# matsengrp/linearham

Hardware: AMD Instinct MI355X
Metric: phylo-HMM log-likelihood evals/sec (100-leaf x 400-site family) (higher is better)
Workload: dtype f64

## Files before the change

linearham_amd/csrc/lh_asr.hip:

```cpp
#include <cstdlib>

#include "lh_device.h"

namespace lh {

namespace {

__device__ __forceinline__ void philox_round(uint32_t& c0, uint32_t& c1, uint32_t& c2, uint32_t& c3, uint32_t k0,
                                             uint32_t k1) {
  const uint64_t p0 = (uint64_t)0xD2511F53u * c0, p1 = (uint64_t)0xCD9E8D57u * c2;
  const uint32_t hi0 = (uint32_t)(p0 >> 32), lo0 = (uint32_t)p0;
  const uint32_t hi1 = (uint32_t)(p1 >> 32), lo1 = (uint32_t)p1;
  const uint32_t n0 = hi1 ^ c1 ^ k0, n2 = hi0 ^ c3 ^ k1;
  c0 = n0;
  c1 = lo1;
  c2 = n2;
  c3 = lo0;
}

__device__ __forceinline__ double asr_uniform(uint64_t seed, uint64_t sample, uint32_t site, uint32_t draw) {
  uint32_t c0 = site, c1 = draw, c2 = (uint32_t)sample, c3 = (uint32_t)(sample >> 32);
  uint32_t k0 = (uint32_t)seed, k1 = (uint32_t)(seed >> 32);
#pragma unroll
  for (int r = 0; r < 10; ++r) {
// ... 190 lines not shown
  uint8_t* flags = st_stack + 16 * 256;
  int32_t* misc = reinterpret_cast<int32_t*>(flags + (((size_t)R * NP + 15) & ~(size_t)15));

  const int tid = threadIdx.x;
  const int lane = tid & 63;
  const int wave = __builtin_amdgcn_readfirstlane(tid >> 6);
  const int n_waves = blockDim.x >> 6;
  const int rate = blockIdx.x;
  const int sample = blockIdx.y;
  const uint64_t sample_id = sample0 + (uint64_t)sample;
  const AsrOp* __restrict__ dsc = desc + (size_t)sample * n_ops;
  const uint8_t* __restrict__ ch = choice_g + (size_t)sample * L;

  for (int i = tid; i < R * NP; i += blockDim.x) flags[i] = 0;
  __syncthreads();
  for (int j = tid; j < L; j += blockDim.x) flags[(int)ch[j] * NP + min(site_pat[j], n_prune)] = 1;
  __syncthreads();

  if (wave == n_waves - 1) {
    int run = 0;
    for (int j0 = 0; j0 < L; j0 += 64) {
      const int j = j0 + lane;
      const int c = j < L ? (int)ch[j] : 255;
      const unsigned long long mine = __ballot(c == rate);
      if (c == rate) list[run + __popcll(mine & ((1ull << lane) - 1ull))] = j;
      run += __popcll(mine);
    }
    int base = 0, prun = 0;
    for (int k = 0; k <= rate; ++k) {
      int cntk = 0;
      for (int p0 = 0; p0 < NP; p0 += 64) {
        const int p = p0 + lane;
        const bool f = p < NP && flags[k * NP + p] != 0;
        const unsigned long long m = __ballot(f);
        if (k == rate && f) {
          const int pos = cntk + __popcll(m & ((1ull << lane) - 1ull));
          plist[pos] = p;
          pslot[p] = pos;
        }
        cntk += __popcll(m);
      }
      if (k < rate)
        base += (cntk + 7) & ~7;
      else
        prun = cntk;
    }
    if (lane == 0) {
      misc[0] = run;
      misc[1] = base;
      misc[2] = prun;
    }
  }

  const double* __restrict__ e = eig + (size_t)sample * 36;
  const double rt = rates[(size_t)sample * R + rate];
  const double* __restrict__ bl = brlen + (size_t)sample * (2 * (size_t)T - 2);
  {
    double P[4][4];
    for (int j = tid; j < T + n_ops - 1; j += blockDim.x) {
      if (j < T) {
        compute_pmatrix(e, bl[j] * rt, P);
        double* o = tiptab + j * 16;
#pragma unroll
        for (int i = 0; i < 4; ++i)
#pragma unroll
          for (int st = 0; st < 4; ++st) o[st * 4 + i] = P[i][st];
      } else {
        const int k = j - T;
        compute_pmatrix(e, bl[T + dsc[k].b.z] * rt, P);
        double* o = pin + (size_t)k * 16;
#pragma unroll
        for (int i = 0; i < 4; ++i)
#pragma unroll
          for (int q = 0; q < 4; ++q) o[i * 4 + q] = P[i][q];
      }
    }
  }
  __syncthreads();
  const int cnt = misc[0], base = misc[1], cntp = misc[2];
  if (cnt == 0) return;

  const double* __restrict__ p4 = pi + (size_t)sample * 4;
  const uint8_t* __restrict__ nv = naive + (size_t)sample * L;
  const size_t plane = (size_t)Lp;
  double2* clv_s = clv + (size_t)sample * n_ops * 2 * plane;
  uint8_t* anc_s = anc + (size_t)sample * n_ops * (size_t)L;
  uint8_t* my_stack = st_stack + tid;

  {
    const int per = 64;
    for (int s0 = wave * per; s0 < cntp; s0 += n_waves * per) {
      const int slot = min(s0 + min(lane, per - 1), cntp - 1);
      const int pat = plist[slot];
      const int gslot = base + slot;
      const bool all_n = pat >= n_prune;
      const unsigned upat = all_n ? 0u : (unsigned)pat;
      const double2* cbase = clv_s + gslot;
      double a[4] = {1.0, 1.0, 1.0, 1.0};
      struct Up {
        int4 da, db;
        int sa, sb;
      };
      Up ring[4];
      double2 ylo[2], yhi[2];
      auto tips = [&](Up& p) {
        p.sa = msa[(unsigned)(p.da.y * n_prune) + upat];
        p.sb = msa[(unsigned)(p.da.z * n_prune) + upat];
// ... 151 lines not shown
```

linearham_amd/csrc/lh_capi.hip:

```cpp
#include <algorithm>
#include <map>
#include <cstdio>
#include <cstring>
#include <atomic>
#include <chrono>
#include <string>
#include <thread>
#include <vector>

#include "lh_device.h"

namespace lh {
const DebugOptions& debug_options() {
  static const DebugOptions opts = [] {
    DebugOptions o;
    auto set = [](const char* name) { return std::getenv(name) != nullptr; };
    auto num = [](const char* name, int dflt) { const char* e = std::getenv(name); return e ? std::atoi(e) : dflt; };
    o.chunk = std::max(256, num("LH_CHUNK", o.chunk));
    o.host_sub = std::max(256, num("LH_HOST_SUB", o.host_sub));
    o.k2b_no_pair = set("LH_K2B_NO_PAIR");
    o.k2b_vd_single = set("LH_K2B_VD_SINGLE");
    o.sample_timing = set("LH_SAMPLE_TIMING");
    o.k1_tile_cap = num("LH_K1_TILE_CAP", 0);
    o.k1_cxx_walk = set("LH_K1_CXX_WALK");
// ... 317 lines not shown
  auto cols = [&](const int32_t* src, size_t rows, size_t n, size_t n_pad, size_t inner) {
    std::vector<int32_t> t = pad_genes<int32_t>(src, rows, n, n_pad, inner, -1);
    for (int32_t& x : t) x = x >= 0 ? remap[x] : n_jcols;
    return t;
  };
  std::vector<double> ltr = pad_genes<double>(j.left_trans, W, nL, pL, 1, 0.0);
  for (size_t l = 0; l < nL; ++l) ltr[l] = j.enter_trans[l];
  std::vector<double> ntt(pR * 16, 0.0);
  for (size_t r = 0; r < nR; ++r)
    for (int a = 0; a < 4; ++a)
      for (int b = 0; b < 4; ++b) ntt[r * 16 + b * 4 + a] = j.right_ntt[r * 16 + a * 4 + b];
  if (upload_vec(f, pad_genes<double>(j.enter_lo, 1, nL, pL, 1, 0.0), &d->enter_lo)) return 1;
  if (upload_vec(f, ltr, &d->left_trans)) return 1;
  if (upload_vec(f, pad_genes<double>(j.left_lo, W, nL, pL, 1, 0.0), &d->left_lo)) return 1;
  if (upload_vec(f, cols(j.left_xmsa, W, nL, pL, 1), &d->left_xmsa)) return 1;
  if (upload_vec(f, pad_genes<double>(j.right_gp_nli, 1, nR, pR, 4, 0.0), &d->right_gp_nli)) return 1;
  if (upload_vec(f, ntt, &d->right_ntt)) return 1;
  if (upload_vec(f, pad_genes<double>(j.right_nlo, W, nR, pR, 4, 0.0), &d->right_nlo)) return 1;
  if (upload_vec(f, pad_genes<double>(j.right_trans, W, nR, pR, 1, 0.0), &d->right_trans)) return 1;
  if (upload_vec(f, pad_genes<double>(j.right_gp_li, W, nR, pR, 1, 0.0), &d->right_gp_li)) return 1;
  if (upload_vec(f, cols(j.right_xmsa, W, nR, pR, 1), &d->right_xmsa)) return 1;
  if (upload_vec(f, cols(j.nti_xmsa, W, nR, pR, 4), &d->nti_xmsa)) return 1;
  if (upload_vec(f, pad_genes<double>(j.exit_nlo, 1, nR, pR, 4, 0.0), &d->exit_nlo)) return 1;
  if (upload_vec(f, pad_genes<double>(j.exit_trans, 1, nR, pR, 1, 0.0), &d->exit_trans)) return 1;
  if (upload_vec(f, pad_genes<double>(j.exit_gp_li, 1, nR, pR, 1, 0.0), &d->exit_gp_li)) return 1;
  std::vector<int32_t> row_pat(W, f->host.n_prune);
  if (xmsa_site)
    for (size_t i = 0; i < W; ++i) row_pat[i] = pat_of_site[xmsa_site[j.nti_xmsa[i * nR * 4]]];
  if (upload_vec(f, row_pat, &d->row_pat)) return 1;
  return 0;
}

size_t k1_bytes_per_sample(const lh_family* f, int T, int R) {
  const lh::PruneWsSizes z = lh::prune_ws_sizes(T, f->host.msa_mixed_n != 0);
  const size_t n_ops = (size_t)std::max(T - 2, 1);
  return sizeof(double) * R * z.scratch_doubles_per_rate + n_ops * (sizeof(int2) + sizeof(double)) +
         z.tabs_per_sample * sizeof(int4) + sizeof(int4);
}

int ensure_workspace(lh_family* f, int n, int R, int T) {
  Workspace& w = f->ws;
  if (n <= w.n_cap && R == w.R && T == w.T) return 0;
  void** bufs[] = {(void**)&w.rates,         (void**)&w.eig,        (void**)&w.site_lik,   (void**)&w.site_scal,
                   (void**)&w.prune.scratch, (void**)&w.prune.wops, (void**)&w.prune.wlen, (void**)&w.prune.tabs,
                   (void**)&w.prune.hdr};
  for (void** b : bufs) {
    if (*b) LH_HIP(hipFree(*b));
    *b = nullptr;
  }
  w.n_cap = 0;
  const size_t L = f->host.n_prune;
  const int cap = std::max(n, 1);
  LH_HIP(hipMalloc((void**)&w.rates, sizeof(double) * cap * R));
  LH_HIP(hipMalloc((void**)&w.eig, sizeof(double) * cap * 36));
  const lh::PruneWsSizes z = lh::prune_ws_sizes(T, f->host.msa_mixed_n != 0);
  const size_t n_ops = (size_t)std::max(T - 2, 1);
  LH_HIP(hipMalloc((void**)&w.prune.scratch, sizeof(double) * cap * R * z.scratch_doubles_per_rate));
  LH_HIP(hipMalloc((void**)&w.prune.wops, sizeof(int2) * cap * n_ops));
  LH_HIP(hipMalloc((void**)&w.prune.wlen, sizeof(double) * cap * n_ops));
  LH_HIP(hipMalloc((void**)&w.prune.tabs, sizeof(int4) * cap * z.tabs_per_sample));
  LH_HIP(hipMalloc((void**)&w.prune.hdr, sizeof(int4) * cap));
  w.prune.err_flag = f->err_flag;
  LH_HIP(hipMalloc((void**)&w.site_lik, sizeof(double) * cap * R * 5 * std::max(L, (size_t)1)));
  LH_HIP(hipMalloc((void**)&w.site_scal, sizeof(int32_t) * cap * R * std::max(L, (size_t)1)));
  w.n_cap = cap;
  w.R = R;
  w.T = T;
  return 0;
}

int stage(lh_family* f, int slot, size_t bytes, void** out) {
  Staging& s = f->st;
  if (bytes > s.cap[slot]) {
    if (s.ptr[slot]) LH_HIP(hipFree(s.ptr[slot]));
    s.ptr[slot] = nullptr;
    s.cap[slot] = 0;
    LH_HIP(hipMalloc(&s.ptr[slot], bytes));
    s.cap[slot] = bytes;
  }
  *out = s.ptr[slot];
  return 0;
}

static const int kChunk = lh::debug_options().chunk;

int run_forward(lh_family* f, int n, int R, const double* site_lik, const int32_t* site_scal, const double* pi,
                const double* em_in, double* em_out, double* loglik_dev, const lh_eval_outputs* outs,
                size_t sample_offset, hipStream_t stream) {
  double* fwd = (outs && outs->forward) ? outs->forward + sample_offset * f->host.forward_size : nullptr;
  int32_t* sco =
      (outs && outs->scaler_counts) ? outs->scaler_counts + sample_offset * f->host.scaler_size : nullptr;
  ForwardWs& w = f->fws;
  if (n > w.n_cap) {
    LH_HIP(hipDeviceSynchronize());
    void** bufs[] = {(void**)&w.gem, (void**)&w.jem, (void**)&w.gcnt, (void**)&w.jrs, (void**)&w.dxf, (void**)&w.dxc};
    for (void** b : bufs) {
      if (*b) LH_HIP(hipFree(*b));
      *b = nullptr;
    }
    w.n_cap = 0;
    LH_HIP(hipMalloc((void**)&w.jrs, sizeof(int32_t) * (size_t)n * std::max(f->host.vd.n_rows + f->host.dj.n_rows, 1)));
    LH_HIP(hipMalloc((void**)&w.dxf, sizeof(double) * (size_t)n * 32));
    LH_HIP(hipMalloc((void**)&w.dxc, sizeof(int32_t) * (size_t)n));
    LH_HIP(hipMalloc((void**)&w.gem, sizeof(double) * (size_t)n * std::max<int64_t>(f->host.gem_size, 1)));
    LH_HIP(hipMalloc((void**)&w.jem, sizeof(double) * (size_t)n * std::max(f->host.n_jcols, 1)));
    LH_HIP(hipMalloc((void**)&w.gcnt, sizeof(int32_t) * (size_t)n * 3));
    w.n_cap = n;
// ... 1208 lines not shown
```

linearham_amd/csrc/lh_device.h:

```cpp
#pragma once
#include <hip/hip_runtime.h>
#include <stdint.h>

#include "linearham_amd.h"

namespace lh {

constexpr double kScaleFactor = 0x1p256;
constexpr double kScaleThreshold = 0x1p-256;
constexpr double kLogScaleFactor = 177.445678223345993274;

enum : int { OP_CHERRY = 0, OP_TIP_ACC = 1, OP_POP_ACC = 2, OP_PUSH_FLAG = 16, OP_RANK_SHIFT = 8 };

enum : int { W_CHERRY = 0, W_TIP_ACC = 1, W_POP = 2, W_CTIP = 3, W_CTAB_ACC = 4 };

struct PruneWs {
  double* scratch;
  int2* wops;
  double* wlen;
  int4* tabs;
  int4* hdr;
  int32_t* err_flag;
};
struct PruneWsSizes {
// ... 50 lines not shown
  DevJunction vd, dj;
  int32_t max_genes;
  int32_t n_jcols;
  const int32_t* jcols;
  int64_t gem_size;
  int64_t forward_size;
  int64_t scaler_size;
};

__device__ static inline double fast_rcp(double v) {
  double r = __builtin_amdgcn_rcp(v);
  r = fma(fma(-v, r, 1.0), r, r);
  r = fma(fma(-v, r, 1.0), r, r);
  return r;
}

struct DevSampleJunction {
  int32_t n_rows, n_left, n_right, n_states;
  int32_t right_first_block;
  const int32_t* state_class;
  const int32_t* left_rows;
  const int32_t* left_dense;
  const double* left_lo;
  const double* left_trans;
  const double* enter_lo;
  const int32_t* right_dense;
  const int32_t* right_first;
  const double* gp;
  const double* nli;
  const double* ntt;
  const double* nlo;
  const double* li;
  const double* rtrans;
  const double* exit_nlo;
  const double* exit_trans;
  const double* exit_li;
  const double* prod;
};

struct DevSampler {
  int32_t has_d, n_v, n_d, n_j, states_per_sample, words_per_sample;
  DevSampleJunction vd, dj;
};

void launch_sample(const DevSampler& smp, const DevSampler* smp_dev, int n, const double* fwd, size_t forward_size, const uint32_t* words,
                   int words_per_sample, int32_t* states, hipStream_t stream);

void launch_posterior(const DevSampler* smp_dev, int n, double* post, size_t forward_size, const double* loglik,
                      hipStream_t stream);
int posterior_slabs(int n);
void launch_posterior_reduce(int n, size_t forward_size, const double* post, const double* loglik, const double* log_offset,
                             double* w, double* partial, double* weighted_sum, double* stats, hipStream_t stream);

__device__ static inline void compute_pmatrix(const double* __restrict__ e, double tr, double P[4][4]) {
  double ex[4];
#pragma unroll
  for (int k = 1; k < 4; ++k) ex[k] = expm1(e[k] * tr);
#pragma unroll
  for (int i = 0; i < 4; ++i)
#pragma unroll
    for (int j = 0; j < 4; ++j) {
      double v = (i == j) ? 1.0 : 0.0;
#pragma unroll
      for (int k = 1; k < 4; ++k) v = fma(e[4 + i * 4 + k] * ex[k], e[20 + k * 4 + j], v);
      P[i][j] = fmax(v, 0.0);
    }
}


void launch_model_setup(int n, int R, const double* er, const double* pi, const double* alpha,
                        double* rates, double* eig, hipStream_t stream);

int launch_prune(const DevFamily& fam, int n, int R, int T, int max_depth, const int32_t* ops,
                 const double* brlen, const double* rates, const double* eig, const PruneWs& ws, const double* pi,
                 double* site_lik, int32_t* site_scal, hipStream_t stream, bool allow_fused = true);
const char* prune_last_form();
const char* prune_last_error();

void launch_gtr_setup(int n, const double* er, const double* pi, double* eig, hipStream_t stream);

int launch_asr(const DevFamily& fam, int n, int R, int T, const int32_t* ops, const double* brlen, const double* rates,
               const double* eig, const double* pi, const double* site_lik, const int32_t* site_scal,
               const uint8_t* naive, uint64_t seed, uint64_t sample0, double* clv, void* desc, uint8_t* anc,
               uint8_t* rate_choice, const int4* hdr , hipStream_t stream);
size_t asr_desc_bytes(int T);
size_t asr_lds_bytes(int T, int L, int R, int n_prune);
size_t asr_slots(int L, int R);

void launch_forward(const DevFamily& fam, const DevFamily* fam_dev, int n, int R, const double* site_lik,
                    const int32_t* site_scal, const double* pi, const double* em_in, double* em_out, double* gem,
                    int32_t* gcnt, double* jem,
                    int32_t* jrs, double* dxf, int32_t* dxc, double* loglik, double* forward_out, int32_t* scaler_out,
                    bool extended, hipStream_t stream);
size_t forward_lds_bytes(const DevFamily& fam);

struct DebugOptions {
  int chunk = 49152;
  int host_sub = 12288;
  bool k2b_no_pair = false;
  bool k2b_vd_single = false;
  bool sample_timing = false;
  int k1_tile_cap = 0;
  bool k1_cxx_walk = false;
  bool k1_tables = false;
  bool k1_stack = false;
  bool k1_no_tables = false;
  bool k1_segments = false;
  int k1_seg_waves = 4;
  bool k1_no_fuse = false;
};
const DebugOptions& debug_options();

}
```

linearham_amd/csrc/lh_model.hip:

```cpp
#include "lh_device.h"

namespace lh {



__device__ static double gamma_p(double a, double x, double lga) {
  if (!(x > 0.0)) return 0.0;
  const double pre = exp(-x + a * log(x) - lga);
  if (x < a + 1.0) {
    double ap = a, del = fast_rcp(a), sum = del;
    for (int n = 0; n < 2000; ++n) {
      ap += 1.0;
      del *= x * fast_rcp(ap);
      sum += del;
      if (fabs(del) < fabs(sum) * 1e-17) break;
    }
    return sum * pre;
  }
  const double FPMIN = 1e-300;
  double b = x + 1.0 - a, c = 1.0 / FPMIN, d = fast_rcp(b), h = d;
  for (int i = 1; i < 2000; ++i) {
    const double an = -i * (i - a);
    b += 2.0;
    d = an * d + b;
// ... 95 lines not shown
  for (int sweep = 0; sweep < 40; ++sweep) {
    double off = 0.0;
    for (int i = 0; i < 4; ++i)
      for (int j = i + 1; j < 4; ++j) off += A[i][j] * A[i][j];
    if (off < 1e-300) break;
#pragma unroll
    for (int pp = 0; pp < 3; ++pp) {
#pragma unroll
      for (int q = pp + 1; q < 4; ++q) {
        const double apq = A[pp][q];
        if (fabs(apq) < 1e-300) continue;
        const double theta = (A[q][q] - A[pp][pp]) / (2.0 * apq);
        const double t = ((theta >= 0.0) ? 1.0 : -1.0) / (fabs(theta) + sqrt(theta * theta + 1.0));
        const double c = 1.0 / sqrt(t * t + 1.0), sn = t * c;
#pragma unroll
        for (int k = 0; k < 4; ++k) {
          const double akp = A[k][pp], akq = A[k][q];
          A[k][pp] = c * akp - sn * akq;
          A[k][q] = sn * akp + c * akq;
        }
#pragma unroll
        for (int k = 0; k < 4; ++k) {
          const double apk = A[pp][k], aqk = A[q][k];
          A[pp][k] = c * apk - sn * aqk;
          A[q][k] = sn * apk + c * aqk;
        }
#pragma unroll
        for (int k = 0; k < 4; ++k) {
          const double wkp = W[k][pp], wkq = W[k][q];
          W[k][pp] = c * wkp - sn * wkq;
          W[k][q] = sn * wkp + c * wkq;
        }
      }
    }
  }
  double lam[4] = {A[0][0], A[1][1], A[2][2], A[3][3]};
#pragma unroll
  for (int k = 3; k >= 1; --k) {
    bool up = true;
#pragma unroll
    for (int j = 0; j < k; ++j) up = up && lam[k] > lam[j];
    if (up) {
      const double t = lam[k];
      lam[k] = lam[k - 1];
      lam[k - 1] = t;
#pragma unroll
      for (int i = 0; i < 4; ++i) {
        const double w = W[i][k];
        W[i][k] = W[i][k - 1];
        W[i][k - 1] = w;
      }
    }
  }
  double* o = eig + (size_t)s * 36;
  o[0] = 0.0;
  for (int k = 1; k < 4; ++k) o[k] = lam[k];
  for (int i = 0; i < 4; ++i)
    for (int k = 0; k < 4; ++k) {
      o[4 + i * 4 + k] = W[i][k] / sq[i];
      o[20 + k * 4 + i] = W[i][k] * sq[i];
    }
}

__global__ void __launch_bounds__(256) finalize_rates_kernel(int n, int R, double* __restrict__ rates) {
  const int s = blockIdx.x * blockDim.x + threadIdx.x;
  if (s >= n) return;
  double* r = rates + (size_t)s * R;
  double prev = 0.0;
  for (int k = 0; k < R - 1; ++k) {
    const double cum = r[k];
    r[k] = (cum - prev) * R;
    prev = cum;
  }
  r[R - 1] = (1.0 - prev) * R;
}

void launch_model_setup(int n, int R, const double* er, const double* pi, const double* alpha,
                        double* rates, double* eig, hipStream_t stream) {
  const long long total = (long long)n * R;
  hipLaunchKernelGGL(model_setup_kernel, dim3((unsigned)((total + 63) / 64)), dim3(64), 0, stream, n, R, er, pi,
                     alpha, rates, eig);
  hipLaunchKernelGGL(finalize_rates_kernel, dim3((n + 255) / 256), dim3(256), 0, stream, n, R, rates);
}

void launch_gtr_setup(int n, const double* er, const double* pi, double* eig, hipStream_t stream) {
  hipLaunchKernelGGL(model_setup_kernel, dim3((unsigned)((n + 63) / 64)), dim3(64), 0, stream, n, 1, er, pi,
                     (const double*)nullptr, (double*)nullptr, eig);
}

}
```

linearham_amd/csrc/lh_prune.hip:

```cpp
#include <cstdlib>

#include <cstdio>

#include "lh_device.h"

namespace lh {

namespace {

thread_local char g_prune_form[64] = "";
thread_local char g_prune_error[256] = "";

#define LH_SLOT_COPY(dst, src)                       \
  _Pragma("unroll") for (int s_ = 0; s_ < S; ++s_) { \
    dst[s_][0] = src[s_][0];                         \
    dst[s_][1] = src[s_][1];                         \
    dst[s_][2] = src[s_][2];                         \
    dst[s_][3] = src[s_][3];                         \
  }
#define LH_PUSH_IF(d)                                   \
  if constexpr (kDepth > d) {                           \
    if (push_mask & (1u << d)) { LH_SLOT_COPY(st##d, a) } \
  }
#define LH_POP_CASE(d)          \
// ... 491 lines not shown
          a[s][0] *= kScaleFactor;
          a[s][1] *= kScaleFactor;
          a[s][2] *= kScaleFactor;
          a[s][3] *= kScaleFactor;
          ++scal[s];
        }
      }
    }
  }
  close_naive_branch<S>(a, scal, naive_tab, p4, lik, scl);
}

#undef LH_SLOT_COPY
#undef LH_PUSH_IF
#undef LH_POP_CASE
#undef LH_POP_SLOT
#undef LH_DECL

}

template <int kDepth, bool kTwo, bool kN, bool kFused, bool kSeg = false>
__device__ __forceinline__ void prune_body(int sample, int n2, int tile, int R, int wpr, const uint8_t* __restrict__ msa, int L,
                                           int T, int n_ops, const int32_t* __restrict__ ops,
                                           const int4* __restrict__ hdr, int32_t* err_flag,
                                           const double* __restrict__ brlen, const double* __restrict__ rates,
                                           const double* __restrict__ eig, double* pmat_w, size_t rate_stride,
                                           const double* __restrict__ pi,
                                           double* __restrict__ site_lik, int32_t* __restrict__ site_scal) {
  extern __shared__ double2 smem2[];
  const int tid = threadIdx.x;
  const int wave_all = __builtin_amdgcn_readfirstlane(tid >> 6);
  const int rate = kFused ? wave_all / wpr : (int)blockIdx.y;
  const int wave = kFused ? wave_all - rate * wpr : wave_all;
  const int nthr = kFused ? wpr * 64 : (int)blockDim.x;
  const int rtid = kFused ? tid - rate * nthr : tid;
  if (hdr != nullptr && hdr[sample].w != 0) {
    const int planes = kFused ? 1 : R, plane = kFused ? 0 : rate;
    const int t0 = blockIdx.x * tile, t1 = min(t0 + tile, L);
    for (int site = t0 + tid; site < t1; site += blockDim.x) {
      for (int b = 0; b < 5; ++b) site_lik[(((size_t)sample * planes + plane) * 5 + b) * (size_t)L + site] = __builtin_nan("");
      site_scal[((size_t)sample * planes + plane) * (size_t)L + site] = 0;
    }
    return;
  }
  const size_t pm_off = ((size_t)sample * R + rate) * rate_stride;
  double* tiptab = reinterpret_cast<double*>(smem2) + (kFused ? (size_t)rate * T * 16 : 0);
  const double* naive_tab = kSeg ? tiptab + 2 * kSegOps * 16 : tiptab;
  double* ones = reinterpret_cast<double*>(smem2) + (kSeg ? (size_t)(2 * kSegOps + 1) * 16 : (size_t)(kFused ? R : 1) * T * 16);
  const int ones_off = (int)(ones - tiptab);
  if (kN && tid < 4) ones[tid] = 1.0;
  const int4* __restrict__ op_ptr = reinterpret_cast<const int4*>(ops) + (size_t)sample * n_ops;

  {
    const double* __restrict__ e = eig + (size_t)sample * 36;
    const double rt = rates[(size_t)sample * R + rate];
    const double* __restrict__ bl = brlen + (size_t)sample * (2 * (size_t)T - 2);
    double* pw = pmat_w + pm_off;
    double P[4][4];
    if constexpr (kFused) {
      uint16_t* mat_list = reinterpret_cast<uint16_t*>(reinterpret_cast<double*>(smem2) + (size_t)R * T * 16 + (kN ? 4 : 0));
      const int nodes = 2 * T - 2;
      if (rate == 0) {
        for (int k = rtid; k < n_ops; k += nthr) {
          const int4 op = op_ptr[k];
          const int kind = op.x & 15, rank = op.x >> OP_RANK_SHIFT;
          if (kind == OP_CHERRY) continue;
          mat_list[rank] = (uint16_t)(2 * k);
          if (kind == OP_POP_ACC) mat_list[rank + 1] = (uint16_t)(2 * k + 1);
        }
      }
      __syncthreads();
      const int n_inner = T - 3;
      for (int it = rtid; it < n_inner + T; it += nthr) {
        if (it < n_inner) {
          const int code = mat_list[it], k = min(code >> 1, n_ops - 1);
          const int4 op = op_ptr[k];
          const int node = min(max((code & 1) ? op.y : op.z, 0), nodes - 1);
          compute_pmatrix(e, bl[node] * rt, P);
          double* o = pw + (size_t)k * 32 + (code & 1) * 16;
#pragma unroll
          for (int i = 0; i < 4; ++i)
#pragma unroll
            for (int q = 0; q < 4; ++q) o[i * 4 + q] = P[i][q];
        } else {
          const int j = it - n_inner;
          compute_pmatrix(e, bl[j] * rt, P);
          double* o = tiptab + j * 16;
#pragma unroll
          for (int i = 0; i < 4; ++i)
#pragma unroll
            for (int st = 0; st < 4; ++st) o[st * 4 + i] = P[i][st];
        }
      }
    } else {
    const int half = nthr >= 128 ? (nthr / 128) * 64 : 0;
    const bool do_ops = half == 0 || rtid < half;
    const bool do_tips = half == 0 || rtid >= half;
    if (do_ops) {
      const int stride = half ? half : nthr;
      for (int k = rtid; k < n_ops; k += stride) {
        const int4 op = op_ptr[k];
        const int kind = op.x & 15;
        if (kind == OP_CHERRY) continue;
        double* o = pw + (size_t)k * 32;
        compute_pmatrix(e, bl[op.z] * rt, P);
#pragma unroll
        for (int i = 0; i < 4; ++i)
#pragma unroll
          for (int q = 0; q < 4; ++q) o[i * 4 + q] = P[i][q];
        if (kind == OP_POP_ACC) {
          compute_pmatrix(e, bl[op.y] * rt, P);
#pragma unroll
          for (int i = 0; i < 4; ++i)
#pragma unroll
            for (int q = 0; q < 4; ++q) o[16 + i * 4 + q] = P[i][q];
        }
      }
    }
    if (do_tips) {
      const int stride = half ? nthr - half : nthr;
      for (int j = half ? rtid - half : rtid; j < (kSeg ? 1 : T); j += stride) {
        compute_pmatrix(e, bl[j] * rt, P);
        double* o = kSeg ? tiptab + 2 * kSegOps * 16 : tiptab + j * 16;
#pragma unroll
        for (int i = 0; i < 4; ++i)
#pragma unroll
          for (int st = 0; st < 4; ++st) o[st * 4 + i] = P[i][st];
      }
    }
    }
  }
  SegCtx seg{eig + (size_t)sample * 36, brlen + (size_t)sample * (2 * (size_t)T - 2),
             rates[(size_t)sample * R + rate], tiptab, rtid, nthr};
  if constexpr (kSeg) seg_fill(seg, op_ptr, n_ops, 0);
  asm volatile("s_waitcnt vmcnt(0)" ::: "memory");
  __threadfence_block();
  __syncthreads();

  const pmat_ptr pm = pmat_after_barrier(pmat_w + pm_off);
  const int lane = tid & 63;
  const int tile0 = blockIdx.x * tile;
  const int site_end = min(tile0 + tile, L);
  const double* __restrict__ p4 = pi + (size_t)sample * 4;
  double lik[2][5];
  int scl[2] = {0, 0};
  int site0, n_own;
  bool two_sites = false;
  if constexpr (kTwo) two_sites = wave < n2;
  if (two_sites) {
    site0 = tile0 + wave * 128 + lane;
    n_own = 2;
    if constexpr (kTwo)
      prune_wave<kDepth, 2, kN, kSeg>(site0, site_end, msa, L, n_ops, op_ptr, pm, tiptab, naive_tab, ones_off, p4, lik, scl, seg);
  } else {
    site0 = tile0 + n2 * 128 + (wave - n2) * 64 + lane;
    n_own = 1;
    double lik1[1][5];
    int scl1[1];
    prune_wave<kDepth, 1, kN, kSeg>(site0, site_end, msa, L, n_ops, op_ptr, pm, tiptab, naive_tab, ones_off, p4, lik1, scl1, seg);
#pragma unroll
    for (int b = 0; b < 5; ++b) lik[0][b] = lik1[0][b];
    scl[0] = scl1[0];
  }

  if constexpr (!kFused) {
    double* lik_out = site_lik + (((size_t)sample * R + rate) * 5) * (size_t)L;
    int32_t* scal_out = site_scal + ((size_t)sample * R + rate) * (size_t)L;
#pragma unroll
    for (int s = 0; s < 2; ++s) {
      const int site = site0 + 64 * s;
      if (s < n_own && site < site_end) {
#pragma unroll
        for (int b = 0; b < 5; ++b) lik_out[(size_t)b * L + site] = lik[s][b];
        scal_out[site] = scl[s];
      }
    }
  } else {
    const int pad = n2 * 128 + (wpr - n2) * 64;
    __syncthreads();
    double* X = reinterpret_cast<double*>(smem2);
    int* SC = reinterpret_cast<int*>(X + (size_t)R * 5 * pad);
#pragma unroll
    for (int s = 0; s < 2; ++s) {
      const int idx = site0 + 64 * s - tile0;
      if (s < n_own && idx < pad) {
// ... 191 lines not shown
      const int up = __shfl_up(incl, d), dup = __shfl_up(dincl, d);
      if (lane >= d) incl += up, dincl += dup;
    }
    const int depth = depth0 + dincl - dl;
    if (in && push && op.w != depth) ok = false;
    if (in && kind == OP_POP_ACC && op.w != depth - 1) ok = false;
    if (check_ranks && in && kind != OP_CHERRY && rank != carry + incl - m) ok = false;
    if (in && !ok) bad = true;
    carry += __shfl(incl, 63);
    depth0 += __shfl(dincl, 63);
  }
  if (carry != T - 3 || depth0 != 0) bad = true;
  const bool any_bad = __builtin_amdgcn_ballot_w64(bad) != 0;
  if (lane == 0) {
    hdr[smp] = make_int4(0, 0, 0, any_bad ? 1 : 0);
    if (any_bad) atomicOr(err_flag, 1);
  }
}

template <int kDepth, bool kN, bool kFused, bool kAsm = false>
__device__ __forceinline__ void prune_body_ct(int n2, int tile, int R, int wpr, const uint8_t* __restrict__ msa,
                                              const uint64_t* __restrict__ planes, int L,
                                              int T, const int2* __restrict__ wops, const double* __restrict__ wlen,
                                              const int4* __restrict__ tabs, int tabs_stride,
                                              const int4* __restrict__ hdr, const double* __restrict__ brlen,
                                              const double* __restrict__ rates, const double* __restrict__ eig,
                                              double* pmat_w, size_t rate_stride, const double* __restrict__ pi,
                                              double* __restrict__ site_lik, int32_t* __restrict__ site_scal) {
  extern __shared__ double2 smem2[];
  constexpr int SY = kN ? 5 : 4, E = SY * SY;
  const int tid = threadIdx.x;
  const int wave_all = __builtin_amdgcn_readfirstlane(tid >> 6);
  const int rate = kFused ? wave_all / wpr : (int)blockIdx.y;
  const int wave = kFused ? wave_all - rate * wpr : wave_all;
  const int nthr = kFused ? wpr * 64 : (int)blockDim.x;
  const int rtid = kFused ? tid - rate * nthr : tid;
  const int sample = blockIdx.z;
  const int n_ops = T - 2;
  const int4 h = hdr[sample];
  const int n_w = __builtin_amdgcn_readfirstlane(h.x);
  const int n_mat = __builtin_amdgcn_readfirstlane(h.y), n_tab = __builtin_amdgcn_readfirstlane(h.z);
  const bool malformed = h.w != 0;
  double* pw = pmat_w + ((size_t)sample * R + rate) * rate_stride;
  double* ctab = pw + (size_t)(T - 3 > 0 ? T - 3 : 0) * 16;
  constexpr int kS = 2;
  double* tiptab = reinterpret_cast<double*>(smem2) + (kFused ? (size_t)rate * T * 16 : 0);
  const double* naive_tab = tiptab;
  double* ones = reinterpret_cast<double*>(smem2) + (size_t)(kFused ? R : 1) * T * 16;
  const int ones_off = (int)(ones - tiptab);
  if (kN && tid < 4) ones[tid] = 1.0;
  const int4* __restrict__ tl = tabs + (size_t)sample * tabs_stride;
  WalkOp* desc = reinterpret_cast<WalkOp*>(reinterpret_cast<double*>(smem2) + (size_t)(kFused ? R : 1) * T * 16 + (kN ? 4 : 0));
  for (int i = tid; i < n_w; i += blockDim.x) desc[i] = wops[(size_t)sample * n_ops + i];

  const int n_q = min(n_tab, nthr >> 2);
  const bool pc_lane = (rtid & 3) == 0 && (rtid >> 2) < n_q;
  int4 tcell = make_int4(1, 1, 0, 0);
  if ((rtid >> 2) < n_q) tcell = tl[rtid >> 2];
  double pcq[16];
#pragma unroll
  for (int i = 0; i < 16; ++i) pcq[i] = 0.0;
  {
    const double* __restrict__ e = eig + (size_t)sample * 36;
    const double* __restrict__ bl = brlen + (size_t)sample * (2 * (size_t)T - 2);
    const double* __restrict__ wl = wlen + (size_t)sample * n_ops;
    const int n_rest = n_tab - n_q;
    const int n_list = n_mat + n_rest + T;
    const int round1 = nthr - n_q;
    auto item = [&](bool is_pc, int it, int rr, int quad) {
      double P[4][4];
      const bool in_list = !is_pc && it < n_list;
      const bool inner = in_list && it < n_mat + n_rest;
      const int slot = it < n_mat ? it : it + n_q;
      const int j = it - (n_mat + n_rest);
      double t = 0.0;
      if (is_pc) t = wl[n_mat + quad];
      else if (inner) t = wl[slot];
      else if (in_list) t = bl[j];
      compute_pmatrix(e, t * rates[(size_t)sample * R + rr], P);
      if (is_pc) {
#pragma unroll
        for (int i = 0; i < 4; ++i)
#pragma unroll
          for (int q = 0; q < 4; ++q) pcq[i * 4 + q] = P[i][q];
      } else if (inner) {
        double* o = pmat_w + ((size_t)sample * R + rr) * rate_stride + (size_t)slot * 16;
#pragma unroll
        for (int i = 0; i < 4; ++i)
#pragma unroll
          for (int q = 0; q < 4; ++q) o[i * 4 + q] = P[i][q];
      } else if (in_list) {
        double* o = reinterpret_cast<double*>(smem2) + (kFused ? (size_t)rr * T * 16 : 0) + j * 16;
#pragma unroll
        for (int i = 0; i < 4; ++i)
#pragma unroll
          for (int st = 0; st < 4; ++st) o[st * 4 + i] = P[i][st];
      }
    };
    const int rem = n_list - round1;
    if (rem > 0) {
      if constexpr (kFused) {
        const float inv_rem = 1.0f / (float)rem;
        for (int c = tid; c < R * rem; c += blockDim.x) {
          int rr = min((int)(((float)c + 0.5f) * inv_rem), R - 1);
          rr -= rr * rem > c ? 1 : 0;
          rr += (rr + 1) * rem <= c ? 1 : 0;
          item(false, round1 + c - rr * rem, rr, 0);
        }
      } else {
        for (int it = round1 + rtid; it < n_list; it += nthr) item(false, it, rate, 0);
      }
    }
    item(pc_lane, rtid - min(n_q, (rtid + 3) >> 2), rate, rtid >> 2);
  }
  if (n_tab > n_q) asm volatile("s_waitcnt vmcnt(0)" ::: "memory");
  asm volatile("s_waitcnt lgkmcnt(0)\n\ts_barrier" ::: "memory");
// ... 183 lines not shown
    LH_PRUNE_SAMPLES((prune_body<kDepth, true, kN, true>))                                           \
  }
LH_PRUNE_KERNEL(prune_kernel_w6, 6)
LH_PRUNE_KERNEL(prune_kernel_w5, 5)
LH_PRUNE_KERNEL(prune_kernel_w4, 4)
#undef LH_PRUNE_KERNEL

template <int kDepth, bool kN>
__global__ void __launch_bounds__(512) __attribute__((amdgpu_waves_per_eu(5, 5))) prune_kernel_seg(LH_PRUNE_PARAMS) {
  LH_PRUNE_SAMPLES((prune_body<kDepth, true, kN, false, true>))
}
template <int kDepth, bool kN>
__global__ void __launch_bounds__(512) __attribute__((amdgpu_waves_per_eu(4, 4))) prune_kernel_seg4(LH_PRUNE_PARAMS) {
  LH_PRUNE_SAMPLES((prune_body<kDepth, true, kN, false, true>))
}

PruneWsSizes prune_ws_sizes(int T, bool mixed_n) {
  PruneWsSizes z;
  z.tabs_per_sample = (size_t)std::max((T - 1) / 2, 1);
  const size_t e = mixed_n ? 25 : 16;
  z.scratch_doubles_per_rate = std::max((size_t)std::max(T - 3, 0) * 16 + z.tabs_per_sample * e * 4, (size_t)std::max(T - 2, 1) * 32);
  return z;
}

int launch_prune(const DevFamily& fam, int n, int R, int T, int max_depth, const int32_t* ops,
                 const double* brlen, const double* rates, const double* eig, const PruneWs& ws, const double* pi,
                 double* site_lik, int32_t* site_scal, hipStream_t stream, bool allow_fused) {
  const int L = fam.n_prune;
  const PruneWsSizes sizes = prune_ws_sizes(T, fam.msa_mixed_n != 0);
  if (L == 0) {
    hipLaunchKernelGGL(schedule_stack_check_kernel, dim3(n), dim3(64), 0, stream, T, std::max(max_depth, 1), 0, ops, ws.hdr, ws.err_flag);
    return R;
  }
  double* pmat = ws.scratch;
  const size_t rate_stride = sizes.scratch_doubles_per_rate;
  const DebugOptions& dbg = debug_options();
  const int cap_env = dbg.k1_tile_cap;
  const int cap = cap_env >= 64 ? std::min(cap_env, 1024) : 1024;
  const int tiles = (L + cap - 1) / cap;
  const int tile = tiles == 1 ? L : (((L + tiles - 1) / tiles + 127) & ~127);
  int n2 = tile / 128, n1;
  {
    const int rem = tile - 128 * n2;
    if (rem > 64) {
      ++n2;
      n1 = 0;
    } else {
      n1 = rem > 0 ? 1 : 0;
    }
  }
  const int wpr = n2 + n1;
  const size_t tip_bytes = (size_t)T * 16 * sizeof(double);
  const size_t pad = (size_t)n2 * 128 + (size_t)n1 * 64;
  const size_t tail_bytes = (((size_t)std::max(T - 2, 1) * sizeof(int2)) + 31) & ~(size_t)15;
  const bool mixed = fam.msa_mixed_n != 0;
  const size_t ones_bytes = mixed ? 32 : 0;
  const size_t fused_lds = std::max((size_t)R * tip_bytes + ones_bytes + tail_bytes, (size_t)R * pad * (5 * sizeof(double) + sizeof(int)));
  const bool fused = allow_fused && !dbg.k1_no_fuse && !dbg.k1_segments &&
                     ((R * wpr <= 8 && fused_lds <= 53 * 1024) ||
                      (R * wpr > 8 && R * wpr <= 16 && fused_lds <= 80 * 1024));
  const bool big = !fused && ((160 * 1024 / tip_bytes) * wpr / 4 < 5 || dbg.k1_segments);
  const bool tables_hook = dbg.k1_tables || dbg.k1_no_tables;
  const bool use_asm = !dbg.k1_cxx_walk;
  const bool stack_fused = fused && max_depth <= 4 && dbg.k1_stack && !tables_hook;
  const bool seg = big && max_depth <= 4 && !tables_hook;
  const size_t seg_bytes = (size_t)(2 * kSegOps + 1) * 16 * sizeof(double) + ones_bytes;
  size_t lds = fused ? fused_lds : seg ? seg_bytes : tip_bytes + ones_bytes + tail_bytes;
  if (lds > 160 * 1024) {
    snprintf(g_prune_error, sizeof(g_prune_error),
             "K1: a tree of %d tips with stack depth %d needs %zu bytes of LDS in the cherry-table form (160 KB per CU)", T, max_depth, lds);
    return -1;
  }
  if (stack_fused || seg) {
    hipLaunchKernelGGL(schedule_stack_check_kernel, dim3(n), dim3(64), 0, stream, T, stack_fused && max_depth <= 3 ? 3 : 4,
                       stack_fused ? 1 : 0, ops, ws.hdr, ws.err_flag);
  } else {
    hipLaunchKernelGGL(schedule_rewrite_kernel, dim3(n), dim3(64), (sizes.tabs_per_sample + 16) * sizeof(int), stream, T, max_depth,
                       (int)sizes.tabs_per_sample, dbg.k1_no_tables ? 0 : 1, ops, brlen, ws.wops, ws.wlen, ws.tabs, ws.hdr, ws.err_flag);
  }
  const int wg_waves = fused ? R * wpr : wpr;
  dim3 grid(tiles, fused ? 1 : R, n), block(64 * wg_waves);
  const int n_ops = T - 2;
  hipError_t attr_rc = hipSuccess;
#define LH_LAUNCH_K(K, NAME)                                                                                     \
  {                                                                                                              \
    if (lds > 64 * 1024)                                                                                         \
      attr_rc = hipFuncSetAttribute(reinterpret_cast<const void*>(K), hipFuncAttributeMaxDynamicSharedMemorySize, (int)lds); \
    snprintf(g_prune_form, sizeof(g_prune_form), "%s", NAME);                                                    \
    if (attr_rc == hipSuccess)                                                                                   \
      hipLaunchKernelGGL(K, grid, block, lds, stream, n, n2, tile, R, wpr, fam.msa, L, T, n_ops, ops, ws.hdr, ws.err_flag, \
                         brlen, rates, eig, pmat, rate_stride, pi, site_lik, site_scal);                        \
  }
#define LH_LAUNCH_CT(K, NAME)                                                                                    \
  {                                                                                                              \
    if (lds > 64 * 1024)                                                                                         \
      attr_rc = hipFuncSetAttribute(reinterpret_cast<const void*>(K), hipFuncAttributeMaxDynamicSharedMemorySize, (int)lds); \
    snprintf(g_prune_form, sizeof(g_prune_form), "%s", NAME);                                                    \
    if (attr_rc == hipSuccess)                                                                                   \
      hipLaunchKernelGGL(K, grid, block, lds, stream, n2, tile, R, wpr, fam.msa, fam.msa_planes, L, T, ws.wops, ws.wlen, ws.tabs, \
                         (int)sizes.tabs_per_sample, ws.hdr, brlen, rates, eig, pmat, rate_stride, pi, site_lik, \
                         site_scal);                                                                             \
  }
  const int lds_waves = lds == 0 ? 8 : (int)((160 * 1024 / lds) * wg_waves / 4);
  if (stack_fused) {
#define LH_LAUNCH_STACK(D, N)                                                          \
  {                                                                                    \
    if (lds_waves >= 6 && D == 3)                                                      \
// ... 78 lines not shown
```

Measured before the change: 8.466 million.

## Precompute symmetric eigen-products and use custom expm1 for P-matrix construction

```diff
diff --git a/linearham_amd/csrc/lh_asr.hip b/linearham_amd/csrc/lh_asr.hip
--- a/linearham_amd/csrc/lh_asr.hip
+++ b/linearham_amd/csrc/lh_asr.hip
@@ -266,7 +266,7 @@
     }
   }
 
-  const double* __restrict__ e = eig + (size_t)sample * 36;
+  const double* __restrict__ e = eig + (size_t)sample * kEigDoubles;
   const double rt = rates[(size_t)sample * R + rate];
   const double* __restrict__ bl = brlen + (size_t)sample * (2 * (size_t)T - 2);
   {
diff --git a/linearham_amd/csrc/lh_capi.hip b/linearham_amd/csrc/lh_capi.hip
--- a/linearham_amd/csrc/lh_capi.hip
+++ b/linearham_amd/csrc/lh_capi.hip
@@ -393,7 +393,7 @@
   const size_t L = f->host.n_prune;
   const int cap = std::max(n, 1);
   LH_HIP(hipMalloc((void**)&w.rates, sizeof(double) * cap * R));
-  LH_HIP(hipMalloc((void**)&w.eig, sizeof(double) * cap * 36));
+  LH_HIP(hipMalloc((void**)&w.eig, sizeof(double) * cap * lh::kEigDoubles));
   const lh::PruneWsSizes z = lh::prune_ws_sizes(T, f->host.msa_mixed_n != 0);
   const size_t n_ops = (size_t)std::max(T - 2, 1);
   LH_HIP(hipMalloc((void**)&w.prune.scratch, sizeof(double) * cap * R * z.scratch_doubles_per_rate));
diff --git a/linearham_amd/csrc/lh_device.h b/linearham_amd/csrc/lh_device.h
--- a/linearham_amd/csrc/lh_device.h
+++ b/linearham_amd/csrc/lh_device.h
@@ -126,19 +126,46 @@
 void launch_posterior_reduce(int n, size_t forward_size, const double* post, const double* loglik, const double* log_offset,
                              double* w, double* partial, double* weighted_sum, double* stats, hipStream_t stream);
 
+__device__ static inline double expm1_nonpos(double x) {
+  x = fmax(x, -40.0);
+  const double kf = __builtin_rint(x * 1.4426950408889634074);
+  double r = fma(kf, -6.93147180369123816490e-01, x);
+  r = fma(kf, -1.90821492927058770002e-10, r);
+  double q = 1.0 / 6227020800.0;
+  q = fma(q, r, 1.0 / 479001600.0);
+  q = fma(q, r, 1.0 / 39916800.0);
+  q = fma(q, r, 1.0 / 3628800.0);
+  q = fma(q, r, 1.0 / 362880.0);
+  q = fma(q, r, 1.0 / 40320.0);
+  q = fma(q, r, 1.0 / 5040.0);
+  q = fma(q, r, 1.0 / 720.0);
+  q = fma(q, r, 1.0 / 120.0);
+  q = fma(q, r, 1.0 / 24.0);
+  q = fma(q, r, 1.0 / 6.0);
+  q = fma(q, r, 0.5);
+  const double p = fma(r * r, q, r);
+  const double s = __builtin_ldexp(1.0, (int)kf);
+  return fma(s, p, s - 1.0);
+}
+
+constexpr int kEigDoubles = 40;
+constexpr int kPairI[10] = {0, 1, 2, 3, 0, 0, 0, 1, 1, 2};
+constexpr int kPairJ[10] = {0, 1, 2, 3, 1, 2, 3, 2, 3, 3};
+
 __device__ static inline void compute_pmatrix(const double* __restrict__ e, double tr, double P[4][4]) {
   double ex[4];
 #pragma unroll
-  for (int k = 1; k < 4; ++k) ex[k] = expm1(e[k] * tr);
+  for (int k = 1; k < 4; ++k) ex[k] = expm1_nonpos(e[k] * tr);
 #pragma unroll
-  for (int i = 0; i < 4; ++i)
+  for (int m = 0; m < 10; ++m) {
+    const int i = kPairI[m], j = kPairJ[m];
+    double v = (i == j) ? 1.0 : 0.0;
 #pragma unroll
-    for (int j = 0; j < 4; ++j) {
-      double v = (i == j) ? 1.0 : 0.0;
-#pragma unroll
-      for (int k = 1; k < 4; ++k) v = fma(e[4 + i * 4 + k] * ex[k], e[20 + k * 4 + j], v);
-      P[i][j] = fmax(v, 0.0);
-    }
+    for (int k = 1; k < 4; ++k) v = fma(e[4 + (k - 1) * 10 + m], ex[k], v);
+    v = fmax(v, 0.0);
+    P[i][j] = v;
+    if (i != j) P[j][i] = v * e[34 + m - 4];
+  }
 }
 
 
diff --git a/linearham_amd/csrc/lh_model.hip b/linearham_amd/csrc/lh_model.hip
--- a/linearham_amd/csrc/lh_model.hip
+++ b/linearham_amd/csrc/lh_model.hip
@@ -171,14 +171,16 @@
       }
     }
   }
-  double* o = eig + (size_t)s * 36;
+  double* o = eig + (size_t)s * kEigDoubles;
   o[0] = 0.0;
   for (int k = 1; k < 4; ++k) o[k] = lam[k];
-  for (int i = 0; i < 4; ++i)
-    for (int k = 0; k < 4; ++k) {
-      o[4 + i * 4 + k] = W[i][k] / sq[i];
-      o[20 + k * 4 + i] = W[i][k] * sq[i];
-    }
+#pragma unroll
+  for (int m = 0; m < 10; ++m) {
+    const int i = kPairI[m], j = kPairJ[m];
+#pragma unroll
+    for (int k = 1; k < 4; ++k) o[4 + (k - 1) * 10 + m] = (W[i][k] / sq[i]) * (W[j][k] * sq[j]);
+    if (i != j) o[34 + m - 4] = p[i] / p[j];
+  }
 }
 
 __global__ void __launch_bounds__(256) finalize_rates_kernel(int n, int R, double* __restrict__ rates) {
@@ -207,4 +209,60 @@
                      (const double*)nullptr, (double*)nullptr, eig);
 }
 
-}
+
+__global__ void expm1_probe_kernel(int n, const double* __restrict__ x, double* __restrict__ y) {
+  const int i = blockIdx.x * blockDim.x + threadIdx.x;
+  if (i < n) y[i] = expm1_nonpos(x[i]);
+}
+
+__global__ void pmatrix_probe_kernel(int n, const double* __restrict__ eig, const double* __restrict__ tr,
+                                     double* __restrict__ P) {
+  const int i = blockIdx.x * blockDim.x + threadIdx.x;
+  if (i >= n) return;
+  double M[4][4];
+  compute_pmatrix(eig + (size_t)i * kEigDoubles, tr[i], M);
+  for (int a = 0; a < 4; ++a)
+    for (int b = 0; b < 4; ++b) P[(size_t)i * 16 + a * 4 + b] = M[a][b];
+}
+
+}
+
+extern "C" int lh_test_expm1_nonpos(int n, const double* x, double* y) {
+  const size_t bytes = sizeof(double) * (size_t)n;
+  double *dx = nullptr, *dy = nullptr;
+  hipError_t e = hipMalloc((void**)&dx, bytes);
+  if (e == hipSuccess) e = hipMalloc((void**)&dy, bytes);
+  if (e == hipSuccess) e = hipMemcpy(dx, x, bytes, hipMemcpyHostToDevice);
+  if (e == hipSuccess && n > 0) {
+    hipLaunchKernelGGL(lh::expm1_probe_kernel, dim3((n + 255) / 256), dim3(256), 0, 0, n, dx, dy);
+    e = hipGetLastError();
+  }
+  if (e == hipSuccess) e = hipMemcpy(y, dy, bytes, hipMemcpyDeviceToHost);
+  (void)hipFree(dx);
+  (void)hipFree(dy);
+  return e == hipSuccess ? 0 : 1;
+}
+
+extern "C" int lh_test_pmatrices(int n, const double* er, const double* pi, const double* tr, double* P) {
+  double *d_er = nullptr, *d_pi = nullptr, *d_tr = nullptr, *d_eig = nullptr, *d_P = nullptr;
+  hipError_t e = hipMalloc((void**)&d_er, sizeof(double) * 6 * (size_t)n);
+  if (e == hipSuccess) e = hipMalloc((void**)&d_pi, sizeof(double) * 4 * (size_t)n);
+  if (e == hipSuccess) e = hipMalloc((void**)&d_tr, sizeof(double) * (size_t)n);
+  if (e == hipSuccess) e = hipMalloc((void**)&d_eig, sizeof(double) * lh::kEigDoubles * (size_t)n);
+  if (e == hipSuccess) e = hipMalloc((void**)&d_P, sizeof(double) * 16 * (size_t)n);
+  if (e == hipSuccess) e = hipMemcpy(d_er, er, sizeof(double) * 6 * (size_t)n, hipMemcpyHostToDevice);
+  if (e == hipSuccess) e = hipMemcpy(d_pi, pi, sizeof(double) * 4 * (size_t)n, hipMemcpyHostToDevice);
+  if (e == hipSuccess) e = hipMemcpy(d_tr, tr, sizeof(double) * (size_t)n, hipMemcpyHostToDevice);
+  if (e == hipSuccess && n > 0) {
+    lh::launch_gtr_setup(n, d_er, d_pi, d_eig, 0);
+    hipLaunchKernelGGL(lh::pmatrix_probe_kernel, dim3((n + 255) / 256), dim3(256), 0, 0, n, d_eig, d_tr, d_P);
+    e = hipGetLastError();
+  }
+  if (e == hipSuccess) e = hipMemcpy(P, d_P, sizeof(double) * 16 * (size_t)n, hipMemcpyDeviceToHost);
+  (void)hipFree(d_er);
+  (void)hipFree(d_pi);
+  (void)hipFree(d_tr);
+  (void)hipFree(d_eig);
+  (void)hipFree(d_P);
+  return e == hipSuccess ? 0 : 1;
+}
diff --git a/linearham_amd/csrc/lh_prune.hip b/linearham_amd/csrc/lh_prune.hip
--- a/linearham_amd/csrc/lh_prune.hip
+++ b/linearham_amd/csrc/lh_prune.hip
@@ -567,7 +567,7 @@
   const int4* __restrict__ op_ptr = reinterpret_cast<const int4*>(ops) + (size_t)sample * n_ops;
 
   {
-    const double* __restrict__ e = eig + (size_t)sample * 36;
+    const double* __restrict__ e = eig + (size_t)sample * kEigDoubles;
     const double rt = rates[(size_t)sample * R + rate];
     const double* __restrict__ bl = brlen + (size_t)sample * (2 * (size_t)T - 2);
     double* pw = pmat_w + pm_off;
@@ -645,7 +645,7 @@
     }
     }
   }
-  SegCtx seg{eig + (size_t)sample * 36, brlen + (size_t)sample * (2 * (size_t)T - 2),
+  SegCtx seg{eig + (size_t)sample * kEigDoubles, brlen + (size_t)sample * (2 * (size_t)T - 2),
              rates[(size_t)sample * R + rate], tiptab, rtid, nthr};
   if constexpr (kSeg) seg_fill(seg, op_ptr, n_ops, 0);
   asm volatile("s_waitcnt vmcnt(0)" ::: "memory");
@@ -943,6 +943,10 @@
   const int4* __restrict__ tl = tabs + (size_t)sample * tabs_stride;
   WalkOp* desc = reinterpret_cast<WalkOp*>(reinterpret_cast<double*>(smem2) + (size_t)(kFused ? R : 1) * T * 16 + (kN ? 4 : 0));
   for (int i = tid; i < n_w; i += blockDim.x) desc[i] = wops[(size_t)sample * n_ops + i];
+  double* e_lds = reinterpret_cast<double*>(reinterpret_cast<char*>(desc) +
+                                            (((size_t)max(n_ops, 1) * sizeof(WalkOp) + 15) & ~(size_t)15));
+  if (tid < kEigDoubles) e_lds[tid] = eig[(size_t)sample * kEigDoubles + tid];
+  __syncthreads();
 
   const int n_q = min(n_tab, nthr >> 2);
   const bool pc_lane = (rtid & 3) == 0 && (rtid >> 2) < n_q;
@@ -952,7 +956,7 @@
 #pragma unroll
   for (int i = 0; i < 16; ++i) pcq[i] = 0.0;
   {
-    const double* __restrict__ e = eig + (size_t)sample * 36;
+    const double* e = e_lds;
     const double* __restrict__ bl = brlen + (size_t)sample * (2 * (size_t)T - 2);
     const double* __restrict__ wl = wlen + (size_t)sample * n_ops;
     const int n_rest = n_tab - n_q;
@@ -1242,7 +1246,7 @@
   const int wpr = n2 + n1;
   const size_t tip_bytes = (size_t)T * 16 * sizeof(double);
   const size_t pad = (size_t)n2 * 128 + (size_t)n1 * 64;
-  const size_t tail_bytes = (((size_t)std::max(T - 2, 1) * sizeof(int2)) + 31) & ~(size_t)15;
+  const size_t tail_bytes = ((((size_t)std::max(T - 2, 1) * sizeof(int2)) + 31) & ~(size_t)15) + kEigDoubles * sizeof(double);
   const bool mixed = fam.msa_mixed_n != 0;
   const size_t ones_bytes = mixed ? 32 : 0;
   const size_t fused_lds = std::max((size_t)R * tip_bytes + ones_bytes + tail_bytes, (size_t)R * pad * (5 * sizeof(double) + sizeof(int)));
```

Result: faster. 8.555 million (median of 6 runs) (+1.0%).
